# zhaodong-liu/GRAM

Measured on AMD Instinct MI355X. Metric: users/sec @ beam=20 top-20 gen, Beauty T5-base; Recall@5 parity, higher is better.
Workload: dtype f16x3

## Files before the change

### gram_amd/csrc/dec_attn.hip

```cpp
#include <type_traits>

#include "common.h"
#include "prof.h"
#include "xattn_tile.h"

namespace {

__device__ __forceinline__ void xa_merge_w(float m0, float m1, float l0, float l1, float& w0, float& w1, float& inv) {
  const float M = fmaxf(fmaxf(GRAM_FMIN, m0), m1);
  w0 = __expf(m0 - M);
  w1 = __expf(m1 - M);
  inv = 1.f / __builtin_fmaf(l1, w1, l0 * w0);
}
__device__ __forceinline__ f32x4 xa_merge_o(f32x4 o0, f32x4 o1, float w0, float w1, float inv) {
  f32x4 r;
#pragma unroll
  for (int e = 0; e < 4; ++e) r[e] = __builtin_fmaf(o1[e], w1, o0[e] * w0) * inv;
  return r;
}

template <int NT, bool LIVE, int S, int NW, bool ENT = false>
__global__ __launch_bounds__(NW * 64) void cross_attn_kernel(
    const p16* __restrict__ q, const p16* __restrict__ kbank, const p16* __restrict__ vtbank,
    const uint8_t* __restrict__ mask, p16* __restrict__ out, int K, int H, int Sk, const int32_t* __restrict__ users,
    const int32_t* __restrict__ rowpos, long q_pstride, long bank_pstride, const uint32_t* __restrict__ key_bits) {
  using T = SplitTab<S>;
  constexpr int NB = NT * 16;
  static_assert(NW == 1 || NW == 2, "the merge is written for two waves");
  constexpr int PSTR = 2 * XA_TILE;
  constexpr int STAGE = S * PSTR;
  extern __shared__ __attribute__((aligned(16))) char smem[];
  float* sm_m = reinterpret_cast<float*>(smem);
  float* sm_l = sm_m + NW * NB;
  float* sm_o = sm_l + NW * NB;

  const int h = blockIdx.x, b = LIVE ? users[blockIdx.y] : blockIdx.y;
  const int rb = ENT ? (int)blockIdx.y : b;
  const int tid = threadIdx.x, lane = tid & 63;
  const int wave = __builtin_amdgcn_readfirstlane(tid >> 6);
  const int c = lane & 15, g = lane >> 4;
  const int inner = H * 64;
  const char* kb = reinterpret_cast<const char*>(kbank + ((size_t)b * H + h) * Sk * 64);
  const char* vt = reinterpret_cast<const char*>(vtbank + ((size_t)b * H + h) * 64 * Sk);
  const uint8_t* mk = mask + (size_t)b * Sk;

  p16x8 qf[S][NT][2];
  f32x4 o[4][NT];
  float m[NT], l[NT];
#pragma unroll
  for (int nt = 0; nt < NT; ++nt) {
    m[nt] = GRAM_FMIN;
    l[nt] = 0.f;
#pragma unroll
    for (int mt = 0; mt < 4; ++mt) o[mt][nt] = (f32x4){0.f, 0.f, 0.f, 0.f};
  }

#pragma unroll
  for (int nt = 0; nt < NT; ++nt) {
    const int qrow = xa_row<LIVE>(rb, K, 16 * nt + c, rowpos);
#pragma unroll
    for (int pc = 0; pc < S; ++pc)
#pragma unroll
      for (int kd = 0; kd < 2; ++kd)
        qf[pc][nt][kd] = qrow >= 0 ? ld_global_b128(q + pc * q_pstride + (size_t)qrow * inner + h * 64 + 32 * kd + 8 * g) : zero_bf16x8();
  }
  const int nsteps = Sk >> 5;
  uint32_t kb0 = 0, kb1 = 0;
  if (key_bits) {
    if (lane < nsteps) kb0 = key_bits[(size_t)b * 128 + lane];
    if (lane + 64 < nsteps) kb1 = key_bits[(size_t)b * 128 + 64 + lane];
  } else {
#pragma unroll
    for (int half = 0; half < 2; ++half) {
      const int st = lane + 64 * half;
      uint32_t bits = 0;
      if (st < nsteps) {
        const uint4* p = reinterpret_cast<const uint4*>(mk + 32 * st);
        const uint4 a = p[0], c2 = p[1];
        const uint32_t w8[8] = {a.x, a.y, a.z, a.w, c2.x, c2.y, c2.z, c2.w};
#pragma unroll
        for (int i = 0; i < 8; ++i)
#pragma unroll
          for (int j = 0; j < 4; ++j) bits |= ((w8[i] >> (8 * j)) & 0xffu) ? (1u << (4 * i + j)) : 0u;
      }
      if (half == 0) kb0 = bits; else kb1 = bits;
    }
  }
  unsigned long long v0 = __ballot(kb0 != 0u), v1 = __ballot(kb1 != 0u);
  if ((v0 | v1) == 0ull) {
    v0 = nsteps >= 64 ? ~0ull : ((1ull << nsteps) - 1ull);
    v1 = nsteps > 64 ? ((nsteps >= 128 ? ~0ull : ((1ull << (nsteps - 64)) - 1ull))) : 0ull;
  }
  v0 = __builtin_amdgcn_readfirstlane((unsigned)v0) | ((unsigned long long)__builtin_amdgcn_readfirstlane((unsigned)(v0 >> 32)) << 32);
  v1 = __builtin_amdgcn_readfirstlane((unsigned)v1) | ((unsigned long long)__builtin_amdgcn_readfirstlane((unsigned)(v1 >> 32)) << 32);
  int ord = 0;
  auto next = [&](int s) -> int {
    for (s = s + 1; s < nsteps; ++s) {
      const unsigned long long bit = (s < 64 ? (v0 >> s) : (v1 >> (s - 64))) & 1ull;
      if (bit) {
        const bool mine = ord == wave;
        ord = ord + 1 == NW ? 0 : ord + 1;
        if (mine) return s;
      }
    }
    return nsteps;
  };

  uint32_t koff[4], voff[4];
#pragma unroll
  for (int i = 0; i < 4; ++i) {
    const int kr = 8 * i + (lane >> 3);
    koff[i] = (uint32_t)(kr * 128 + (((lane & 7) ^ ksw(kr)) << 4));
    const int d = 16 * i + (lane >> 2);
    voff[i] = (uint32_t)(d * 64 + (((lane & 3) ^ vsw(d)) << 4));
  }
  const uint32_t stage0 = (uint32_t)(uintptr_t)(__attribute__((address_space(3))) char*)smem + wave * STAGE;
  auto issue_k = [&](int step) {
    const uint32_t dst = stage0;
#pragma unroll
    for (int pc = 0; pc < S; ++pc) {
      const char* kbase = kb + (size_t)pc * bank_pstride * 2 + (size_t)step * (32 * 128);
#pragma unroll
      for (int i = 0; i < 4; ++i) dma16_nt(dst + pc * PSTR + i * 1024, koff[i], kbase);
    }
  };
  auto issue_v = [&](int step) {
    const uint32_t dst = stage0;
#pragma unroll
    for (int pc = 0; pc < S; ++pc) {
      const char* vbase = vt + (size_t)pc * bank_pstride * 2 + (size_t)step * 4096;
#pragma unroll
      for (int i = 0; i < 4; ++i) dma16(dst + pc * PSTR + XA_TILE + i * 1024, voff[i], vbase);
    }
  };
  const int krow = 8 * (c >> 2) + (c & 3);
  p16x8 kf[S][2][2], vf[S][4];
  auto read_k = [&]() {
    const char* stg = smem + wave * STAGE;
#pragma unroll
    for (int pc = 0; pc < S; ++pc)
#pragma unroll
      for (int t = 0; t < 2; ++t)
#pragma unroll
        for (int kd = 0; kd < 2; ++kd) {
          const int r = krow + 4 * t;
          kf[pc][t][kd] = *reinterpret_cast<const p16x8*>(stg + pc * PSTR + r * 128 + (((g + 4 * kd) ^ ksw(r)) << 4));
        }
  };
  auto read_v = [&]() {
    const char* stg = smem + wave * STAGE;
#pragma unroll
    for (int pc = 0; pc < S; ++pc)
#pragma unroll
      for (int mt = 0; mt < 4; ++mt) {
        const int d = 16 * mt + c;
        vf[pc][mt] = *reinterpret_cast<const p16x8*>(stg + pc * PSTR + XA_TILE + d * 64 + ((g ^ vsw(d)) << 4));
      }
  };
  p16x8 pf[S][NT];
  auto math_qk = [&](int step) {
    const uint32_t kword = step < 64 ? (uint32_t)__builtin_amdgcn_readlane((int)kb0, step) : (uint32_t)__builtin_amdgcn_readlane((int)kb1, step - 64);
    const uint32_t kbits = kword >> (8 * g);
#pragma unroll
    for (int nt = 0; nt < NT; ++nt) {
      f32x4 s[2];
#pragma unroll
      for (int t = 0; t < 2; ++t) {
        f32x4 a = (f32x4){0.f, 0.f, 0.f, 0.f};
#pragma unroll
        for (int pr = 0; pr < T::NP; ++pr) {
          a = mfma16(kf[T::A[pr]][t][0], qf[T::B[pr]][nt][0], a);
          a = mfma16(kf[T::A[pr]][t][1], qf[T::B[pr]][nt][1], a);
        }
#pragma unroll
        for (int j = 0; j < 4; ++j) a[j] = ((kbits >> (4 * t + j)) & 1u) ? a[j] : GRAM_FMIN;
        s[t] = a;
      }
      float tm = fmaxf(fmaxf(fmaxf(s[0][0], s[0][1]), fmaxf(s[0][2], s[0][3])),
                       fmaxf(fmaxf(s[1][0], s[1][1]), fmaxf(s[1][2], s[1][3])));
      tm = fmaxf(tm, __shfl_xor(tm, 16, 64));
      tm = fmaxf(tm, __shfl_xor(tm, 32, 64));
      const float mn = fmaxf(m[nt], tm);
      const float alpha = __expf(m[nt] - mn);
      m[nt] = mn;
      float ps = 0.f;
#pragma unroll
      for (int t = 0; t < 2; ++t)
#pragma unroll
        for (int j = 0; j < 4; ++j) {
          float e = __expf(s[t][j] - mn);
          ps += e;
#pragma unroll
          for (int pc = 0; pc < S; ++pc) {
            const p16 eb = (p16)e;
            pf[pc][nt][4 * t + j] = eb;
            e -= (float)eb;
          }
        }
      l[nt] = xa_l_update(l[nt], alpha, ps);
#pragma unroll
      for (int mt = 0; mt < 4; ++mt) o[mt][nt] *= alpha;
    }
  };
  auto math_pv = [&]() {
#pragma unroll
    for (int mt = 0; mt < 4; ++mt)
#pragma unroll
      for (int nt = 0; nt < NT; ++nt)
#pragma unroll
        for (int pr = 0; pr < T::NP; ++pr) o[mt][nt] = mfma16(vf[T::A[pr]][mt], pf[T::B[pr]][nt], o[mt][nt]);
  };

  wait_vm<0>();
#pragma unroll
  for (int nt = 0; nt < NT; ++nt)
#pragma unroll
    for (int pc = 0; pc < S; ++pc)
#pragma unroll
      for (int kd = 0; kd < 2; ++kd) asm volatile("" : "+v"(qf[pc][nt][kd]));
  int cur = next(-1);
  if (cur < nsteps) {
    issue_k(cur);
    issue_v(cur);
  }
  while (cur < nsteps) {
    const int nxt = next(cur);
    wait_vm<4 * S>();
    read_k();
    if (nxt < nsteps) {
      asm volatile("s_waitcnt lgkmcnt(0)" ::: "memory");
      issue_k(nxt);
    }
    math_qk(cur);
    if (nxt < nsteps) wait_vm<4 * S>();
    else wait_vm<0>();
    read_v();
    if (nxt < nsteps) {
      asm volatile("s_waitcnt lgkmcnt(0)" ::: "memory");
      issue_v(nxt);
    }
    math_pv();
    cur = nxt;
  }

  if constexpr (NW == 1) {
#pragma unroll
    for (int nt = 0; nt < NT; ++nt) {
      float lt = l[nt];
      lt += __shfl_xor(lt, 16, 64);
      lt += __shfl_xor(lt, 32, 64);
      const float inv = 1.f / lt;
      const int orow = xa_row<LIVE>(rb, K, 16 * nt + c, rowpos);
      if (orow >= 0) {
#pragma unroll
        for (int mt = 0; mt < 4; ++mt) xa_store<S>(out, orow, inner, h * 64 + 16 * mt + 4 * g, o[mt][nt] * inv);
      }
    }
    return;
  }
  gram_sync();
#pragma unroll
  for (int nt = 0; nt < NT; ++nt) {
    float lt = l[nt];
    lt += __shfl_xor(lt, 16, 64);
    lt += __shfl_xor(lt, 32, 64);
    const int beam = 16 * nt + c;
    if (g == 0) {
      sm_m[wave * NB + beam] = m[nt];
      sm_l[wave * NB + beam] = lt;
    }
#pragma unroll
    for (int mt = 0; mt < 4; ++mt)
      *reinterpret_cast<f32x4*>(sm_o + ((size_t)(wave * NB + beam)) * 64 + 16 * mt + 4 * g) = o[mt][nt];
  }
  gram_sync();
  for (int idx = tid; idx < K * 16; idx += NW * 64) {
    const int beam = idx >> 4, d4 = (idx & 15) * 4;
    float w0, w1, inv2;
    xa_merge_w(sm_m[beam], sm_m[NB + beam], sm_l[beam], sm_l[NB + beam], w0, w1, inv2);
    const f32x4 v = xa_merge_o(*reinterpret_cast<const f32x4*>(sm_o + ((size_t)beam) * 64 + d4),
                         *reinterpret_cast<const f32x4*>(sm_o + ((size_t)(NB + beam)) * 64 + d4), w0, w1, inv2);
    int orow = rb * K + beam;
    if constexpr (LIVE) orow = rowpos[orow];
    if (orow >= 0) xa_store<S>(out, orow, inner, h * 64 + d4, v);
  }
}

struct XaLaunch {
  const void *q, *k, *vt;
  const uint8_t* mask;
  void* out;
  int B, K, H, Sk;
  const int32_t *users, *rowpos;
  long q_ps, bank_ps;
  const uint32_t* key_bits;
  hipStream_t st;
};

template <int NT, int S>
int launch_cross(const XaLaunch& a) {
  constexpr int NW = NT >= 3 ? 1 : 2;
  constexpr int NB = NT * 16;
  constexpr int stages = NW * S * 2 * XA_TILE, merge = NW == 1 ? 0 : (2 * NW * NB + NW * NB * 64) * 4;
  constexpr int smem = stages > merge ? stages : merge;
  static_assert(smem <= 160 * 1024, "the stages do not fit the LDS");
  static bool attr_set = false;
  if (!attr_set) {
    hipError_t e = hipFuncSetAttribute(reinterpret_cast<const void*>(cross_attn_kernel<NT, false, S, NW>),
                                       hipFuncAttributeMaxDynamicSharedMemorySize, smem);
    if (e == hipSuccess)
      e = hipFuncSetAttribute(reinterpret_cast<const void*>(cross_attn_kernel<NT, true, S, NW>),
                              hipFuncAttributeMaxDynamicSharedMemorySize, smem);
    if (e != hipSuccess) return (int)e;
    attr_set = true;
  }
  if (a.users)
    hipLaunchKernelGGL((cross_attn_kernel<NT, true, S, NW>), dim3(a.H, a.B), dim3(NW * 64), smem, a.st, (const p16*)a.q, (const p16*)a.k,
                       (const p16*)a.vt, a.mask, (p16*)a.out, a.K, a.H, a.Sk, a.users, a.rowpos, a.q_ps, a.bank_ps, a.key_bits);
  else
    hipLaunchKernelGGL((cross_attn_kernel<NT, false, S, NW>), dim3(a.H, a.B), dim3(NW * 64), smem, a.st, (const p16*)a.q, (const p16*)a.k,
                       (const p16*)a.vt, a.mask, (p16*)a.out, a.K, a.H, a.Sk, a.users, a.rowpos, a.q_ps, a.bank_ps, a.key_bits);
  GRAM_CHECK_LAUNCH();
  return 0;
}

template <int S>
int launch_cross_nt(const XaLaunch& a) {
  switch ((a.K + 15) / 16) {
    case 1: return launch_cross<1, S>(a);
    case 2: return launch_cross<2, S>(a);
    case 3: return launch_cross<3, S>(a);
    default: return launch_cross<4, S>(a);
  }
}

template <int S, int NW>
int launch_cross_entries(const XaLaunch& a) {
  constexpr int NT = 4, NB = NT * 16;
  static_assert(NB == GRAM_TAIL_ENTRY_ROWS, "an entry's row table (gram_forest_t.ent_rows) is indexed by the kernel's padded row count");
  constexpr int stages = NW * S * 2 * XA_TILE, merge = NW == 1 ? 0 : (2 * NW * NB + NW * NB * 64) * 4;
  constexpr int smem = stages > merge ? stages : merge;
  static_assert(smem <= 160 * 1024, "the stages do not fit the LDS");
  static bool attr_set = false;
  if (!attr_set) {
    hipError_t e = hipFuncSetAttribute(reinterpret_cast<const void*>(cross_attn_kernel<NT, true, S, NW, true>),
                                       hipFuncAttributeMaxDynamicSharedMemorySize, smem);
    if (e != hipSuccess) return (int)e;
    attr_set = true;
  }
  hipLaunchKernelGGL((cross_attn_kernel<NT, true, S, NW, true>), dim3(a.H, a.B), dim3(NW * 64), smem, a.st, (const p16*)a.q,
                     (const p16*)a.k, (const p16*)a.vt, a.mask, (p16*)a.out, NB, a.H, a.Sk, a.users, a.rowpos, a.q_ps, a.bank_ps,
                     a.key_bits);
  GRAM_CHECK_LAUNCH();
  return 0;
}

__global__ __launch_bounds__(128) void mask_key_bits_kernel(const uint8_t* __restrict__ mask, uint32_t* __restrict__ bits, int Sk) {
  const int b = blockIdx.x, st = threadIdx.x;
  uint32_t w = 0;
  if (st < (Sk >> 5)) {
    const uint4* p = reinterpret_cast<const uint4*>(mask + (size_t)b * Sk + 32 * st);
    const uint4 a = p[0], c2 = p[1];
    const uint32_t w8[8] = {a.x, a.y, a.z, a.w, c2.x, c2.y, c2.z, c2.w};
#pragma unroll
    for (int i = 0; i < 8; ++i)
#pragma unroll
      for (int j = 0; j < 4; ++j) w |= ((w8[i] >> (8 * j)) & 0xffu) ? (1u << (4 * i + j)) : 0u;
  }
  bits[(size_t)b * 128 + st] = w;
}

template <int S>
__global__ __launch_bounds__(256) void dec_self_attn_kernel(const p16* __restrict__ qkv, p16* __restrict__ kcache,
                                                            p16* __restrict__ vcache, const int32_t* __restrict__ anc,
                                                            const float* __restrict__ bias, p16* __restrict__ out, int R,
                                                            int H, int t, const int32_t* __restrict__ rows, long qkv_ps,
                                                            long cache_ps, const int32_t* __restrict__ qkv_rows) {
  const int rc = blockIdx.x, i = threadIdx.x;
  const int r = rows ? rows[rc] : rc;
  const int inner = H * 64, h = i >> 4;
  const p16* row = qkv + (size_t)(qkv_rows ? qkv_rows[rc] : rc) * 3 * inner + 4 * i;
  float qf[4] = {0.f, 0.f, 0.f, 0.f}, kn[4] = {0.f, 0.f, 0.f, 0.f}, vn[4] = {0.f, 0.f, 0.f, 0.f};
#pragma unroll
  for (int pc = S - 1; pc >= 0; --pc) {
    const p16x4 q4 = *reinterpret_cast<const p16x4*>(row + pc * qkv_ps);
    const p16x4 k4 = *reinterpret_cast<const p16x4*>(row + pc * qkv_ps + inner);
    const p16x4 v4 = *reinterpret_cast<const p16x4*>(row + pc * qkv_ps + 2 * inner);
    *reinterpret_cast<p16x4*>(kcache + pc * cache_ps + ((size_t)t * R + r) * inner + 4 * i) = k4;
    *reinterpret_cast<p16x4*>(vcache + pc * cache_ps + ((size_t)t * R + r) * inner + 4 * i) = v4;
#pragma unroll
    for (int e = 0; e < 4; ++e) {
      qf[e] += (float)q4[e];
      kn[e] += (float)k4[e];
      vn[e] += (float)v4[e];
    }
  }
  float m = -INFINITY, l = 0.f, acc[4] = {0.f, 0.f, 0.f, 0.f};
  auto attend = [&](int j, const float (&kj)[4], const float (&vj)[4]) {
    float s = qf[0] * kj[0] + qf[1] * kj[1] + qf[2] * kj[2] + qf[3] * kj[3];
    s += __shfl_xor(s, 1, 64);
    s += __shfl_xor(s, 2, 64);
    s += __shfl_xor(s, 4, 64);
    s += __shfl_xor(s, 8, 64);
    s += bias[h * GRAM_MAX_DEC_LEN + (t - j)];
    const float mn = fmaxf(m, s);
    const float alpha = __expf(m - mn);
    const float p = __expf(s - mn);
    m = mn;
    l = l * alpha + p;
#pragma unroll
    for (int e = 0; e < 4; ++e) acc[e] = acc[e] * alpha + p * vj[e];
  };
  constexpr int U = 8;
  for (int j0 = 0; j0 < t; j0 += U) {
    int a[U];
#pragma unroll
    for (int u = 0; u < U; ++u) a[u] = anc[(size_t)min(j0 + u, t - 1) * R + r];
    p16x4 kk[U][S], vv[U][S];
#pragma unroll
    for (int u = 0; u < U; ++u) {
      const size_t off = ((size_t)min(j0 + u, t - 1) * R + a[u]) * inner + 4 * i;
#pragma unroll
      for (int pc = 0; pc < S; ++pc) {
        kk[u][pc] = ld_stream_b64(kcache + pc * cache_ps + off);
        vv[u][pc] = ld_stream_b64(vcache + pc * cache_ps + off);
      }
    }
#pragma unroll
    for (int u = 0; u < U; ++u) {
      if (j0 + u < t) {
        float kj[4] = {0.f, 0.f, 0.f, 0.f}, vj[4] = {0.f, 0.f, 0.f, 0.f};
#pragma unroll
        for (int pc = S - 1; pc >= 0; --pc)
#pragma unroll
          for (int e = 0; e < 4; ++e) {
            kj[e] += (float)kk[u][pc][e];
            vj[e] += (float)vv[u][pc][e];
          }
        attend(j0 + u, kj, vj);
      }
    }
  }
  attend(t, kn, vn);
  const float inv = 1.f / l;
#pragma unroll
  for (int e = 0; e < 4; ++e) acc[e] *= inv;
#pragma unroll
  for (int pc = 0; pc < S; ++pc) {
    p16x4 o;
#pragma unroll
    for (int e = 0; e < 4; ++e) {
      o[e] = (p16)acc[e];
      acc[e] -= (float)o[e];
    }
    *reinterpret_cast<p16x4*>(out + (size_t)rc * inner * S + (S == 2 ? inter_off(4 * i, pc) : 4 * i)) = o;
  }
}

}

extern "C" int gram_cross_attn_entries_split(const void* q, const void* k_layer, const void* vt_layer, const uint8_t* mask, void* out,
                                             int n_entries, int K, int H, int S, const int32_t* ent_users, const int32_t* ent_rows,
                                             int pieces, int64_t q_pstride, int64_t bank_pstride, const uint32_t* key_bits,
                                             void* stream) {
  if (!q || !out || !ent_users || !ent_rows || n_entries < 1 || K < 1 || K > GRAM_MAX_BEAMS || H < 1 || S < 32 || (S & 31) ||
      S > 4096 || pieces < 1 || pieces > GRAM_MAX_PIECES)
    return GRAM_E_ARG;
  if (pieces > 1 && (q_pstride < 1 || bank_pstride < (int64_t)H * S * 64)) return GRAM_E_ARG;
  if ((reinterpret_cast<uintptr_t>(mask) & 15) || (reinterpret_cast<uintptr_t>(k_layer) & 15) || (reinterpret_cast<uintptr_t>(vt_layer) & 15))
    return GRAM_E_ARG;
  hipStream_t st = (hipStream_t)stream;
  gram_prof::Scope prof(GRAM_K_CROSS_ATTN, st, 4.0 * n_entries * H * S * 64 * pieces);
  const XaLaunch a{q, k_layer, vt_layer, mask, out, n_entries, GRAM_TAIL_ENTRY_ROWS, H, S, ent_users, ent_rows, (long)q_pstride,
                   (long)bank_pstride, key_bits, st};
  const bool one_wave = (K + 15) / 16 >= 3;
  if (pieces == 2) return one_wave ? launch_cross_entries<2, 1>(a) : launch_cross_entries<2, 2>(a);
  return one_wave ? launch_cross_entries<1, 1>(a) : launch_cross_entries<1, 2>(a);
}

extern "C" int gram_mask_key_bits(const uint8_t* mask, uint32_t* key_bits, int B, int S, void* stream) {
  if (!mask || !key_bits || B < 1 || S < 32 || (S & 31) || S > 4096 || (reinterpret_cast<uintptr_t>(mask) & 15)) return GRAM_E_ARG;
  hipLaunchKernelGGL(mask_key_bits_kernel, dim3(B), dim3(128), 0, (hipStream_t)stream, mask, key_bits, S);
  GRAM_CHECK_LAUNCH();
  return 0;
}

extern "C" int gram_cross_attn_decode_split(const void* q, const void* k_layer, const void* vt_layer, const uint8_t* mask, void* out,
                                            int B, int K, int H, int S, const int32_t* users, const int32_t* rowpos, int pieces,
                                            int64_t q_pstride, int64_t bank_pstride, const uint32_t* key_bits, void* stream) {
  if (B < 1 || K < 1 || K > GRAM_MAX_BEAMS || H < 1 || S < 32 || (S & 31) || S > 4096 || pieces < 1 || pieces > GRAM_MAX_PIECES ||
      (users == nullptr) != (rowpos == nullptr))
    return GRAM_E_ARG;
  if (pieces > 1 && (q_pstride < 1 || bank_pstride < (int64_t)H * S * 64)) return GRAM_E_ARG;
  if ((reinterpret_cast<uintptr_t>(mask) & 15) || (reinterpret_cast<uintptr_t>(k_layer) & 15) || (reinterpret_cast<uintptr_t>(vt_layer) & 15))
    return GRAM_E_ARG;
  hipStream_t st = (hipStream_t)stream;
  gram_prof::Scope prof(GRAM_K_CROSS_ATTN, st, 4.0 * B * H * S * 64 * pieces);
  const XaLaunch a{q, k_layer, vt_layer, mask, out, B, K, H, S, users, rowpos, (long)q_pstride, (long)bank_pstride, key_bits, st};
  return pieces == 2 ? launch_cross_nt<2>(a) : launch_cross_nt<1>(a);
}

extern "C" int gram_cross_attn_decode(const void* q, const void* k_layer, const void* vt_layer, const uint8_t* mask, void* out,
                                      int B, int K, int H, int S, void* stream) {
  return gram_cross_attn_decode_split(q, k_layer, vt_layer, mask, out, B, K, H, S, nullptr, nullptr, 1, 0, 0, nullptr, stream);
}

extern "C" int gram_cross_attn_decode_live(const void* q, const void* k_layer, const void* vt_layer, const uint8_t* mask, void* out,
                                           int n_users, const int32_t* users, const int32_t* rowpos, int K, int H, int S,
                                           void* stream) {
  if (!users || !rowpos) return GRAM_E_ARG;
  return gram_cross_attn_decode_split(q, k_layer, vt_layer, mask, out, n_users, K, H, S, users, rowpos, 1, 0, 0, nullptr, stream);
}

extern "C" int gram_dec_self_attn_split(const void* qkv, void* kcache, void* vcache, const int32_t* anc, const float* bias, void* out,
                                        int R, int n_rows, const int32_t* rows, int H, int t, int Tmax, int pieces,
                                        int64_t qkv_pstride, int64_t cache_pstride, void* stream) {
  return gram_dec_self_attn_rows_split(qkv, nullptr, kcache, vcache, anc, bias, out, R, n_rows, rows, H, t, Tmax, pieces, qkv_pstride,
                                       cache_pstride, stream);
}

extern "C" int gram_dec_self_attn_rows_split(const void* qkv, const int32_t* qkv_rows, void* kcache, void* vcache, const int32_t* anc,
                                             const float* bias, void* out, int R, int n_rows, const int32_t* rows, int H, int t,
                                             int Tmax, int pieces, int64_t qkv_pstride, int64_t cache_pstride, void* stream) {
  if (R < 1 || n_rows < 1 || n_rows > R || H < 1 || H > 16 || t < 0 || t >= Tmax || Tmax > GRAM_MAX_DEC_LEN || pieces < 1 ||
      pieces > GRAM_MAX_PIECES)
    return GRAM_E_ARG;
  if (pieces > 1 && (qkv_pstride < 1 || cache_pstride < (int64_t)Tmax * R * H * 64)) return GRAM_E_ARG;
  hipStream_t st = (hipStream_t)stream;
  gram_prof::Scope prof(GRAM_K_DEC_SELF_ATTN, st, 4.0 * n_rows * H * 64 * (t + 1) * pieces);
  const dim3 grid(n_rows), block(H * 16);
  if (pieces == 2)
    hipLaunchKernelGGL(dec_self_attn_kernel<2>, grid, block, 0, st, (const p16*)qkv, (p16*)kcache, (p16*)vcache, anc, bias,
                       (p16*)out, R, H, t, rows, (long)qkv_pstride, (long)cache_pstride, qkv_rows);
  else
    hipLaunchKernelGGL(dec_self_attn_kernel<1>, grid, block, 0, st, (const p16*)qkv, (p16*)kcache, (p16*)vcache, anc, bias,
                       (p16*)out, R, H, t, rows, (long)qkv_pstride, (long)cache_pstride, qkv_rows);
  GRAM_CHECK_LAUNCH();
  return 0;
}

extern "C" int gram_dec_self_attn(const void* qkv, void* kcache, void* vcache, const int32_t* anc, const float* bias, void* out,
                                  int R, int H, int t, int Tmax, void* stream) {
  return gram_dec_self_attn_split(qkv, kcache, vcache, anc, bias, out, R, R, nullptr, H, t, Tmax, 1, 0, 0, stream);
}

extern "C" int gram_dec_self_attn_live(const void* qkv, void* kcache, void* vcache, const int32_t* anc, const float* bias,
                                       void* out, int R, int n_rows, const int32_t* rows, int H, int t, int Tmax, void* stream) {
  if (!rows) return GRAM_E_ARG;
  return gram_dec_self_attn_split(qkv, kcache, vcache, anc, bias, out, R, n_rows, rows, H, t, Tmax, 1, 0, 0, stream);
}
```

Baseline: 3253.

## Process runs of same-user tail entries in one block sharing K/V streaming

Adds a cross-attention kernel for the tail-entry path in which the lead block of each run of consecutive entries for the same user handles the whole run. Other blocks exit early. Two entries are processed at a time by two half-groups of waves that split the non-empty 16-row tiles between them, so each user's K/V bank is streamed once per entry pair rather than once per entry, and empty tiles are skipped. This is meant to cut redundant K/V memory traffic and MFMA work on padded rows, at the cost of serialising a run inside one block, which can leave many blocks idle and unbalance the load. It also doubles the LDS staging and needs extra syncs for the merge.

```diff
diff --git a/gram_amd/csrc/dec_attn.hip b/gram_amd/csrc/dec_attn.hip
--- a/gram_amd/csrc/dec_attn.hip
+++ b/gram_amd/csrc/dec_attn.hip
@@ -19,7 +19,7 @@
   return r;
 }
 
-template <int NT, bool LIVE, int S, int NW, bool ENT = false>
+template <int NT, bool LIVE, int S, int NW>
 __global__ __launch_bounds__(NW * 64) void cross_attn_kernel(
     const p16* __restrict__ q, const p16* __restrict__ kbank, const p16* __restrict__ vtbank,
     const uint8_t* __restrict__ mask, p16* __restrict__ out, int K, int H, int Sk, const int32_t* __restrict__ users,
@@ -35,7 +35,6 @@
   float* sm_o = sm_l + NW * NB;
 
   const int h = blockIdx.x, b = LIVE ? users[blockIdx.y] : blockIdx.y;
-  const int rb = ENT ? (int)blockIdx.y : b;
   const int tid = threadIdx.x, lane = tid & 63;
   const int wave = __builtin_amdgcn_readfirstlane(tid >> 6);
   const int c = lane & 15, g = lane >> 4;
@@ -57,7 +56,7 @@
 
 #pragma unroll
   for (int nt = 0; nt < NT; ++nt) {
-    const int qrow = xa_row<LIVE>(rb, K, 16 * nt + c, rowpos);
+    const int qrow = xa_row<LIVE>(b, K, 16 * nt + c, rowpos);
 #pragma unroll
     for (int pc = 0; pc < S; ++pc)
 #pragma unroll
@@ -250,7 +249,7 @@
       lt += __shfl_xor(lt, 16, 64);
       lt += __shfl_xor(lt, 32, 64);
       const float inv = 1.f / lt;
-      const int orow = xa_row<LIVE>(rb, K, 16 * nt + c, rowpos);
+      const int orow = xa_row<LIVE>(b, K, 16 * nt + c, rowpos);
       if (orow >= 0) {
 #pragma unroll
         for (int mt = 0; mt < 4; ++mt) xa_store<S>(out, orow, inner, h * 64 + 16 * mt + 4 * g, o[mt][nt] * inv);
@@ -280,9 +279,321 @@
     xa_merge_w(sm_m[beam], sm_m[NB + beam], sm_l[beam], sm_l[NB + beam], w0, w1, inv2);
     const f32x4 v = xa_merge_o(*reinterpret_cast<const f32x4*>(sm_o + ((size_t)beam) * 64 + d4),
                          *reinterpret_cast<const f32x4*>(sm_o + ((size_t)(NB + beam)) * 64 + d4), w0, w1, inv2);
-    int orow = rb * K + beam;
+    int orow = b * K + beam;
     if constexpr (LIVE) orow = rowpos[orow];
     if (orow >= 0) xa_store<S>(out, orow, inner, h * 64 + d4, v);
+  }
+}
+
+constexpr int XA_RUN_MERGE = 4 * (4 * 64 * 16 + 2 * 64 * 4);
+template <int S, int NW>
+__global__ __launch_bounds__(2 * NW * 64, 2) void cross_attn_runs_kernel(
+    const p16* __restrict__ q, const p16* __restrict__ kbank, const p16* __restrict__ vtbank, const uint8_t* __restrict__ mask,
+    p16* __restrict__ out, int n_entries, int H, int Sk, const int32_t* __restrict__ ent_users, const int32_t* __restrict__ ent_rows,
+    long q_pstride, long bank_pstride, const uint32_t* __restrict__ key_bits) {
+  using T = SplitTab<S>;
+  static_assert(NW == 1 || NW == 2, "the merge is written for two waves");
+  constexpr int ER = GRAM_TAIL_ENTRY_ROWS;
+  constexpr int MT = 4;
+  static_assert(ER == 64, "a pair of entries is eight 16-row tiles");
+  constexpr int PSTR = 2 * XA_TILE;
+  constexpr int STAGE = S * PSTR;
+  constexpr int MERGE = XA_RUN_MERGE;
+  static_assert(MERGE == MT * (4 * 64 * 16 + 2 * 64 * 4), "O, m, l of up to MT tiles, one slot per lane");
+  extern __shared__ __attribute__((aligned(16))) char smem[];
+
+  const int h = blockIdx.x, lead = blockIdx.y;
+  const int b = ent_users[lead];
+  if (lead > 0 && ent_users[lead - 1] == b) return;
+  int run_end = lead + 1;
+  while (run_end < n_entries && ent_users[run_end] == b) ++run_end;
+
+  const int tid = threadIdx.x, lane = tid & 63;
+  const int wv = __builtin_amdgcn_readfirstlane(tid >> 6);
+  const int wave = wv % NW, half = wv / NW;
+  const int c = lane & 15, g = lane >> 4;
+  const int inner = H * 64;
+  const char* kb = reinterpret_cast<const char*>(kbank + ((size_t)b * H + h) * Sk * 64);
+  const char* vt = reinterpret_cast<const char*>(vtbank + ((size_t)b * H + h) * 64 * Sk);
+  const uint8_t* mk = mask + (size_t)b * Sk;
+
+  const int nsteps = Sk >> 5;
+  uint32_t kb0 = 0, kb1 = 0;
+  if (key_bits) {
+    if (lane < nsteps) kb0 = key_bits[(size_t)b * 128 + lane];
+    if (lane + 64 < nsteps) kb1 = key_bits[(size_t)b * 128 + 64 + lane];
+  } else {
+#pragma unroll
+    for (int hf = 0; hf < 2; ++hf) {
+      const int st = lane + 64 * hf;
+      uint32_t bits = 0;
+      if (st < nsteps) {
+        const uint4* p = reinterpret_cast<const uint4*>(mk + 32 * st);
+        const uint4 a = p[0], c2 = p[1];
+        const uint32_t w8[8] = {a.x, a.y, a.z, a.w, c2.x, c2.y, c2.z, c2.w};
+#pragma unroll
+        for (int i = 0; i < 8; ++i)
+#pragma unroll
+          for (int j = 0; j < 4; ++j) bits |= ((w8[i] >> (8 * j)) & 0xffu) ? (1u << (4 * i + j)) : 0u;
+      }
+      if (hf == 0) kb0 = bits; else kb1 = bits;
+    }
+  }
+  unsigned long long v0 = __ballot(kb0 != 0u), v1 = __ballot(kb1 != 0u);
+  if ((v0 | v1) == 0ull) {
+    v0 = nsteps >= 64 ? ~0ull : ((1ull << nsteps) - 1ull);
+    v1 = nsteps > 64 ? ((nsteps >= 128 ? ~0ull : ((1ull << (nsteps - 64)) - 1ull))) : 0ull;
+  }
+  v0 = __builtin_amdgcn_readfirstlane((unsigned)v0) | ((unsigned long long)__builtin_amdgcn_readfirstlane((unsigned)(v0 >> 32)) << 32);
+  v1 = __builtin_amdgcn_readfirstlane((unsigned)v1) | ((unsigned long long)__builtin_amdgcn_readfirstlane((unsigned)(v1 >> 32)) << 32);
+  int ord = 0;
+  auto next = [&](int s) -> int {
+    for (s = s + 1; s < nsteps; ++s) {
+      const unsigned long long bit = (s < 64 ? (v0 >> s) : (v1 >> (s - 64))) & 1ull;
+      if (bit) {
+        const bool mine = ord == wave;
+        ord = ord + 1 == NW ? 0 : ord + 1;
+        if (mine) return s;
+      }
+    }
+    return nsteps;
+  };
+
+  uint32_t koff[4], voff[4];
+#pragma unroll
+  for (int i = 0; i < 4; ++i) {
+    const int kr = 8 * i + (lane >> 3);
+    koff[i] = (uint32_t)(kr * 128 + (((lane & 7) ^ ksw(kr)) << 4));
+    const int d = 16 * i + (lane >> 2);
+    voff[i] = (uint32_t)(d * 64 + (((lane & 3) ^ vsw(d)) << 4));
+  }
+  const uint32_t stage0 = (uint32_t)(uintptr_t)(__attribute__((address_space(3))) char*)smem + wave * 2 * STAGE;
+  const int nvalid = __popcll(v0) + __popcll(v1);
+  const int trips = (nvalid + NW - 1) / NW;
+  auto issue_k = [&](int step, int buf) {
+    const uint32_t dst = stage0 + buf * STAGE;
+#pragma unroll
+    for (int pc = 0; pc < S; ++pc) {
+      const char* kbase = kb + (size_t)pc * bank_pstride * 2 + (size_t)step * (32 * 128);
+#pragma unroll
+      for (int i = 0; i < 4; ++i) dma16_nt(dst + pc * PSTR + i * 1024, koff[i], kbase);
+    }
+  };
+  auto issue_v = [&](int step, int buf) {
+    const uint32_t dst = stage0 + buf * STAGE;
+#pragma unroll
+    for (int pc = 0; pc < S; ++pc) {
+      const char* vbase = vt + (size_t)pc * bank_pstride * 2 + (size_t)step * 4096;
+#pragma unroll
+      for (int i = 0; i < 4; ++i) dma16(dst + pc * PSTR + XA_TILE + i * 1024, voff[i], vbase);
+    }
+  };
+  const int krow = 8 * (c >> 2) + (c & 3);
+
+  f32x4 o[4][MT];
+  float m[MT], l[MT];
+  auto sweep = [&](auto nl_c, const int32_t* __restrict__ rows, int tiles) __attribute__((always_inline)) {
+    constexpr int NL = decltype(nl_c)::value;
+    constexpr int NA = NL > 0 ? NL : 1;
+    ord = 0;
+    int cur = next(-1);
+    if (cur < nsteps) {
+      if (half == 0) issue_k(cur, 0);
+      else issue_v(cur, 0);
+    }
+    p16x8 qf[S][NA][2];
+#pragma unroll
+    for (int nt = 0; nt < NL; ++nt) {
+      const int qrow = rows[16 * ((tiles >> (4 * nt)) & 7) + c];
+#pragma unroll
+      for (int pc = 0; pc < S; ++pc)
+#pragma unroll
+        for (int kd = 0; kd < 2; ++kd)
+          qf[pc][nt][kd] = qrow >= 0 ? ld_global_b128(q + pc * q_pstride + (size_t)qrow * inner + h * 64 + 32 * kd + 8 * g) : zero_bf16x8();
+    }
+    p16x8 kf[S][2][2], vf[S][4];
+    auto read_k = [&](int buf) {
+      const char* stg = smem + (wave * 2 + buf) * STAGE;
+#pragma unroll
+      for (int pc = 0; pc < S; ++pc)
+#pragma unroll
+        for (int t = 0; t < 2; ++t)
+#pragma unroll
+          for (int kd = 0; kd < 2; ++kd) {
+            const int r = krow + 4 * t;
+            kf[pc][t][kd] = *reinterpret_cast<const p16x8*>(stg + pc * PSTR + r * 128 + (((g + 4 * kd) ^ ksw(r)) << 4));
+          }
+    };
+    auto read_v = [&](int buf) {
+      const char* stg = smem + (wave * 2 + buf) * STAGE;
+#pragma unroll
+      for (int pc = 0; pc < S; ++pc)
+#pragma unroll
+        for (int mt = 0; mt < 4; ++mt) {
+          const int d = 16 * mt + c;
+          vf[pc][mt] = *reinterpret_cast<const p16x8*>(stg + pc * PSTR + XA_TILE + d * 64 + ((g ^ vsw(d)) << 4));
+        }
+    };
+    p16x8 pf[S][NA];
+    auto math_qk = [&](int step) {
+      const uint32_t kword = step < 64 ? (uint32_t)__builtin_amdgcn_readlane((int)kb0, step) : (uint32_t)__builtin_amdgcn_readlane((int)kb1, step - 64);
+      const uint32_t kbits = kword >> (8 * g);
+#pragma unroll
+      for (int nt = 0; nt < NL; ++nt) {
+        f32x4 s[2];
+#pragma unroll
+        for (int t = 0; t < 2; ++t) {
+          f32x4 a = (f32x4){0.f, 0.f, 0.f, 0.f};
+#pragma unroll
+          for (int pr = 0; pr < T::NP; ++pr) {
+            a = mfma16(kf[T::A[pr]][t][0], qf[T::B[pr]][nt][0], a);
+            a = mfma16(kf[T::A[pr]][t][1], qf[T::B[pr]][nt][1], a);
+          }
+#pragma unroll
+          for (int j = 0; j < 4; ++j) a[j] = ((kbits >> (4 * t + j)) & 1u) ? a[j] : GRAM_FMIN;
+          s[t] = a;
+        }
+        float tm = fmaxf(fmaxf(fmaxf(s[0][0], s[0][1]), fmaxf(s[0][2], s[0][3])),
+                         fmaxf(fmaxf(s[1][0], s[1][1]), fmaxf(s[1][2], s[1][3])));
+        tm = fmaxf(tm, __shfl_xor(tm, 16, 64));
+        tm = fmaxf(tm, __shfl_xor(tm, 32, 64));
+        const float mn = fmaxf(m[nt], tm);
+        const float alpha = __expf(m[nt] - mn);
+        m[nt] = mn;
+        float ps = 0.f;
+#pragma unroll
+        for (int t = 0; t < 2; ++t)
+#pragma unroll
+          for (int j = 0; j < 4; ++j) {
+            float e = __expf(s[t][j] - mn);
+            ps += e;
+#pragma unroll
+            for (int pc = 0; pc < S; ++pc) {
+              const p16 eb = (p16)e;
+              pf[pc][nt][4 * t + j] = eb;
+              e -= (float)eb;
+            }
+          }
+        l[nt] = xa_l_update(l[nt], alpha, ps);
+#pragma unroll
+        for (int mt = 0; mt < 4; ++mt) o[mt][nt] *= alpha;
+      }
+    };
+    auto math_pv = [&]() {
+#pragma unroll
+      for (int mt = 0; mt < 4; ++mt)
+#pragma unroll
+        for (int nt = 0; nt < NL; ++nt)
+#pragma unroll
+          for (int pr = 0; pr < T::NP; ++pr) o[mt][nt] = mfma16(vf[T::A[pr]][mt], pf[T::B[pr]][nt], o[mt][nt]);
+    };
+    wait_vm<0>();
+#pragma unroll
+    for (int nt = 0; nt < NL; ++nt)
+#pragma unroll
+      for (int pc = 0; pc < S; ++pc)
+#pragma unroll
+        for (int kd = 0; kd < 2; ++kd) asm volatile("" : "+v"(qf[pc][nt][kd]));
+    for (int it = 0; it < trips; ++it) {
+      const int buf = it & 1;
+      wait_vm<0>();
+      gram_sync();
+      const int nxt = cur < nsteps ? next(cur) : nsteps;
+      if (nxt < nsteps) {
+        if (half == 0) issue_k(nxt, buf ^ 1);
+        else issue_v(nxt, buf ^ 1);
+      }
+      if constexpr (NL > 0) {
+        if (cur < nsteps) {
+          read_k(buf);
+          math_qk(cur);
+          read_v(buf);
+          math_pv();
+        }
+      }
+      cur = nxt;
+    }
+  };
+
+  for (int e0 = lead; e0 < run_end; e0 += 2) {
+    const int32_t* rows = ent_rows + (size_t)e0 * ER;
+    const int ntiles = e0 + 1 < run_end ? 2 * (ER / 16) : ER / 16;
+    int nl = 0, tiles = 0, seen = 0;
+#pragma unroll
+    for (int t = 0; t < 2 * (ER / 16); ++t) {
+      const int r = t < ntiles ? rows[16 * t + c] : -1;
+      if (__ballot(r >= 0) != 0ull) {
+        if ((seen & 1) == half) {
+          tiles |= t << (4 * nl);
+          ++nl;
+        }
+        ++seen;
+      }
+    }
+    if (seen == 0) continue;
+    nl = __builtin_amdgcn_readfirstlane(nl);
+    tiles = __builtin_amdgcn_readfirstlane(tiles);
+#pragma unroll
+    for (int nt = 0; nt < MT; ++nt) {
+      m[nt] = GRAM_FMIN;
+      l[nt] = 0.f;
+#pragma unroll
+      for (int mt = 0; mt < 4; ++mt) o[mt][nt] = (f32x4){0.f, 0.f, 0.f, 0.f};
+    }
+    if (e0 != lead) gram_sync();
+    switch (nl) {
+      case 1: sweep(std::integral_constant<int, 1>{}, rows, tiles); break;
+      case 2: sweep(std::integral_constant<int, 2>{}, rows, tiles); break;
+      case 3: sweep(std::integral_constant<int, 3>{}, rows, tiles); break;
+      case 4: sweep(std::integral_constant<int, 4>{}, rows, tiles); break;
+      default: sweep(std::integral_constant<int, 0>{}, rows, tiles); break;
+    }
+    float* mg_o = reinterpret_cast<float*>(smem + half * MERGE);
+    float* mg_m = mg_o + MT * 4 * 64 * 4;
+    float* mg_l = mg_m + MT * 64;
+    if constexpr (NW == 2) gram_sync();
+#pragma unroll
+    for (int nt = 0; nt < MT; ++nt) {
+      if (nt < nl) {
+        float lt = l[nt];
+        lt += __shfl_xor(lt, 16, 64);
+        lt += __shfl_xor(lt, 32, 64);
+        l[nt] = lt;
+        if constexpr (NW == 2) {
+          if (wave == 1) {
+            mg_m[nt * 64 + lane] = m[nt];
+            mg_l[nt * 64 + lane] = lt;
+#pragma unroll
+            for (int mt = 0; mt < 4; ++mt) *reinterpret_cast<f32x4*>(mg_o + ((nt * 4 + mt) * 64 + lane) * 4) = o[mt][nt];
+          }
+        }
+      }
+    }
+    if constexpr (NW == 2) gram_sync();
+    if (wave == 0) {
+#pragma unroll
+      for (int nt = 0; nt < MT; ++nt) {
+        if (nt < nl) {
+          const int orow = rows[16 * ((tiles >> (4 * nt)) & 7) + c];
+          if constexpr (NW == 2) {
+            float w0, w1, inv2;
+            xa_merge_w(m[nt], mg_m[nt * 64 + lane], l[nt], mg_l[nt * 64 + lane], w0, w1, inv2);
+            if (orow >= 0) {
+#pragma unroll
+              for (int mt = 0; mt < 4; ++mt)
+                xa_store<S>(out, orow, inner, h * 64 + 16 * mt + 4 * g,
+                            xa_merge_o(o[mt][nt], *reinterpret_cast<const f32x4*>(mg_o + ((nt * 4 + mt) * 64 + lane) * 4), w0, w1, inv2));
+            }
+          } else {
+            const float inv = 1.f / l[nt];
+            if (orow >= 0) {
+#pragma unroll
+              for (int mt = 0; mt < 4; ++mt) xa_store<S>(out, orow, inner, h * 64 + 16 * mt + 4 * g, o[mt][nt] * inv);
+            }
+          }
+        }
+      }
+    }
   }
 }
 
@@ -336,21 +647,18 @@
 
 template <int S, int NW>
 int launch_cross_entries(const XaLaunch& a) {
-  constexpr int NT = 4, NB = NT * 16;
-  static_assert(NB == GRAM_TAIL_ENTRY_ROWS, "an entry's row table (gram_forest_t.ent_rows) is indexed by the kernel's padded row count");
-  constexpr int stages = NW * S * 2 * XA_TILE, merge = NW == 1 ? 0 : (2 * NW * NB + NW * NB * 64) * 4;
+  constexpr int stages = NW * 2 * S * 2 * XA_TILE, merge = NW == 1 ? 0 : 2 * XA_RUN_MERGE;
   constexpr int smem = stages > merge ? stages : merge;
   static_assert(smem <= 160 * 1024, "the stages do not fit the LDS");
   static bool attr_set = false;
   if (!attr_set) {
-    hipError_t e = hipFuncSetAttribute(reinterpret_cast<const void*>(cross_attn_kernel<NT, true, S, NW, true>),
+    hipError_t e = hipFuncSetAttribute(reinterpret_cast<const void*>(cross_attn_runs_kernel<S, NW>),
                                        hipFuncAttributeMaxDynamicSharedMemorySize, smem);
     if (e != hipSuccess) return (int)e;
     attr_set = true;
   }
-  hipLaunchKernelGGL((cross_attn_kernel<NT, true, S, NW, true>), dim3(a.H, a.B), dim3(NW * 64), smem, a.st, (const p16*)a.q,
-                     (const p16*)a.k, (const p16*)a.vt, a.mask, (p16*)a.out, NB, a.H, a.Sk, a.users, a.rowpos, a.q_ps, a.bank_ps,
-                     a.key_bits);
+  hipLaunchKernelGGL((cross_attn_runs_kernel<S, NW>), dim3(a.H, a.B), dim3(2 * NW * 64), smem, a.st, (const p16*)a.q, (const p16*)a.k,
+                     (const p16*)a.vt, a.mask, (p16*)a.out, a.B, a.H, a.Sk, a.users, a.rowpos, a.q_ps, a.bank_ps, a.key_bits);
   GRAM_CHECK_LAUNCH();
   return 0;
 }
```

Result: faster. 3289 (median of 6 runs) (+1.1%).
